# yukiteruono/pbsim3

Measured on AMD Instinct MI355X. Metric: simulated bases/sec, higher is better.
Workload: dtype u8

## Files before the change

pbsim3_amd/csrc/deflate_host.cpp:

```cpp
#include <hip/hip_runtime.h>
#include <limits.h>
#include <math.h>
#include <stdio.h>
#include <stdlib.h>
#include <string.h>

#include <algorithm>
#include <chrono>
#include <functional>
#include <memory>
#include <string>
#include <thread>
#include <vector>

#include "ctx.h"
#include "engine_internal.h"
#include "unit_io.h"

extern "C" {

extern "C++" {
namespace {

int ensure_deflate_tables(pbsim_ctx *c) {
// ... 250 lines not shown
}

}
}

extern "C++" int pbsim::deflate_pieces(pbsim_ctx *c, DfLane &lane, const uint8_t *d_text, int64_t n,
                                       const std::function<int(const char *, int64_t)> &consume,
                                       const std::function<char *(int64_t)> *place, const std::function<bool()> *tail_hook) {
  return deflate_stream(c, lane, d_text, n, consume, place, tail_hook);
}
extern "C++" int pbsim::deflate_handoff(pbsim_ctx *c, DfLane &next, int lane_index, const uint8_t *d_text, int64_t n,
                                        bool own_staging, hipEvent_t text_ready) {
  hipStream_t st = c->df_streams[lane_index][0];
  if (!st || next.own_streams || next.hand_open || n <= 0) return fail("deflate_handoff: bad argument");
  if (!next.ev_hand) HIP_OK(hipEventCreateWithFlags(&next.ev_hand, hipEventDisableTiming));
  HIP_OK(hipStreamWaitEvent(st, text_ready, 0));
  const int ok = df_begin(c, next, d_text, n, own_staging, nullptr);
  if (!ok) next.pre_valid = false;
  next.hand_open = true;
  HIP_OK(hipEventRecord(next.ev_hand, st));
  return ok;
}
extern "C++" int pbsim::deflate_settle(DfLane &lane) {
  if (!lane.hand_open) return PBSIM_SUCCEEDED;
  lane.pre_valid = false;
  HIP_OK(hipEventSynchronize(lane.ev_hand));
  lane.hand_open = false;
  return PBSIM_SUCCEEDED;
}
extern "C++" int pbsim::ensure_deflate_ready(pbsim_ctx *c) {
  for (auto &lane : c->df_streams)
    for (hipStream_t &st : lane)
      if (!st) HIP_OK(hipStreamCreateWithFlags(&st, hipStreamNonBlocking));
  return ensure_deflate_tables(c);
}
extern "C++" int pbsim::ensure_crc_tables(pbsim_ctx *c) { return ensure_deflate_tables(c); }
extern "C++" int pbsim::deflate_prelaunch(pbsim_ctx *c, Slot &sl, bool want_read, bool want_maf) {
  const pbsim_batch_info &bi = sl.b_info;
  if (want_read && bi.read_text_bytes > 0 && !df_begin(c, sl.df[0], sl.d_read_text.as<uint8_t>(), bi.read_text_bytes, true, sl.stream))
    return PBSIM_FAILED;
  if (want_maf && bi.maf_text_bytes > 0 && !df_begin(c, sl.df[1], sl.d_maf_text.as<uint8_t>(), bi.maf_text_bytes, true, sl.stream))
    return PBSIM_FAILED;
  return PBSIM_SUCCEEDED;
}

int pbsim_set_deflate(pbsim_ctx *c, int on) {
  if (!c) return fail("bad argument");
  c->deflate = on & 3;
  c->deflate_parallel = (on & 4) != 0;
  return PBSIM_SUCCEEDED;
}

int64_t pbsim_deflate_bound(int64_t n) {
  if (n <= 0) return 0;
  return n + ((n + DF_CHUNK - 1) / DF_CHUNK) * 31;
}

int pbsim_batch_fetch_deflated(pbsim_ctx *c, char *read_gz, int64_t read_cap, char *maf_gz, int64_t maf_cap,
                               int64_t *read_gz_bytes, int64_t *maf_gz_bytes) {
  if (!c || !c->s().b_finalized) return fail("pbsim_batch_fetch_deflated: no finalized batch");
  NEED_DEVICE(c);
  HIP_OK(hipSetDevice(c->device));
  int64_t nr = 0, nm = 0;
  if (read_gz && !deflate_to_host(c, c->s().df[0], c->s().d_read_text.as<uint8_t>(), c->s().b_info.read_text_bytes, read_gz,
                                  read_cap, &nr))
    return PBSIM_FAILED;
  if (maf_gz && !deflate_to_host(c, c->s().df[0], c->s().d_maf_text.as<uint8_t>(), c->s().b_info.maf_text_bytes, maf_gz,
                                 maf_cap, &nm))
    return PBSIM_FAILED;
  if (read_gz_bytes) *read_gz_bytes = nr;
  if (maf_gz_bytes) *maf_gz_bytes = nm;
  return PBSIM_SUCCEEDED;
}

int pbsim_deflate_buffer(pbsim_ctx *c, const void *src, int64_t n, void *dst, int64_t cap, int64_t *out_bytes) {
  if (!c || !out_bytes || n < 0 || (n > 0 && (!src || !dst))) return fail("pbsim_deflate_buffer: bad argument");
  NEED_DEVICE(c);
  HIP_OK(hipSetDevice(c->device));
  *out_bytes = 0;
  if (n == 0) return PBSIM_SUCCEEDED;
  Slot &sl = c->slots[0];
  DevBuf d_in;
  HIP_OK(d_in.ensure((size_t)n + 16));
  HIP_OK(hipMemcpyAsync(d_in.p, src, (size_t)n, hipMemcpyHostToDevice, sl.stream));
  HIP_OK(hipStreamSynchronize(sl.stream));
  return deflate_to_host(c, sl.df[0], d_in.as<uint8_t>(), n, (char *)dst, cap, out_bytes);
}

extern "C++" int pbsim::deliver(pbsim_ctx *c, const pbsim_sink *sink) {
  const pbsim_batch_info &bi = c->s().b_info;
  if (sink && c->defer_text_sync) {
    NEED_DEVICE(c);
    HIP_OK(hipEventSynchronize(c->s().ev_text));
  }
  if (sink && c->deflate) {
    const bool zr = c->deflate & 1, zm = c->deflate & 2;
    NEED_DEVICE(c);
    HIP_OK(hipSetDevice(c->device));
    if (!zr) HIP_OK(c->s().h_read_text.ensure((size_t)bi.read_text_bytes + 16));
    if (!zm) HIP_OK(c->s().h_maf_text.ensure((size_t)bi.maf_text_bytes + 16));
    if ((!zr || !zm) &&
        !pbsim_batch_fetch(c, zr ? nullptr : (char *)c->s().h_read_text.p, zm ? nullptr : (char *)c->s().h_maf_text.p))
      return PBSIM_FAILED;
    Slot &sl = c->s();
    auto send_read = [&]() -> int {
      if (!(sink->on_read_text && bi.read_text_bytes)) return PBSIM_SUCCEEDED;
      if (!zr)
        return sink->on_read_text(sink->user, (const char *)sl.h_read_text.p, bi.read_text_bytes) ? PBSIM_SUCCEEDED
                                                                                                 : fail("sink aborted (read text)");
      return deflate_stream(c, sl.df[0], sl.d_read_text.as<uint8_t>(), bi.read_text_bytes, [&](const char *z, int64_t k) {
        return sink->on_read_text(sink->user, z, k) ? PBSIM_SUCCEEDED : fail("sink aborted (read text)");
      });
    };
    auto send_maf = [&]() -> int {
      if (!(sink->on_maf_text && bi.maf_text_bytes)) return PBSIM_SUCCEEDED;
      if (!zm)
        return sink->on_maf_text(sink->user, (const char *)sl.h_maf_text.p, bi.maf_text_bytes) ? PBSIM_SUCCEEDED
                                                                                              : fail("sink aborted (MAF text)");
      return deflate_stream(c, sl.df[1], sl.d_maf_text.as<uint8_t>(), bi.maf_text_bytes, [&](const char *z, int64_t k) {
        return sink->on_maf_text(sink->user, z, k) ? PBSIM_SUCCEEDED : fail("sink aborted (MAF text)");
      });
    };
    if (c->deflate_parallel && zr && zm && bi.read_text_bytes && bi.maf_text_bytes) {
      if (!ensure_deflate_tables(c)) return PBSIM_FAILED;
      int ok_read = PBSIM_SUCCEEDED;
      std::string err_read;
      std::thread t([&]() {
        (void)hipSetDevice(c->device);
        ok_read = send_read();
        if (!ok_read) err_read = g_err;
      });
      const int ok_maf = send_maf();
      t.join();
      if (!ok_read) return fail(err_read);
      if (!ok_maf) return PBSIM_FAILED;
    } else {
      if (!send_read()) return PBSIM_FAILED;
      if (!send_maf()) return PBSIM_FAILED;
    }
  } else if (sink) {
    HIP_OK(c->s().h_read_text.ensure((size_t)bi.read_text_bytes + 16));
    HIP_OK(c->s().h_maf_text.ensure((size_t)bi.maf_text_bytes + 16));
    if (!pbsim_batch_fetch(c, (char *)c->s().h_read_text.p, (char *)c->s().h_maf_text.p)) return PBSIM_FAILED;
    if (sink->on_read_text && bi.read_text_bytes &&
        !sink->on_read_text(sink->user, (const char *)c->s().h_read_text.p, bi.read_text_bytes))
      return fail("sink aborted (read text)");
    if (sink->on_maf_text && bi.maf_text_bytes &&
        !sink->on_maf_text(sink->user, (const char *)c->s().h_maf_text.p, bi.maf_text_bytes))
      return fail("sink aborted (MAF text)");
  }
  return c->defer_account ? PBSIM_SUCCEEDED : pbsim_batch_account(c);
}
}
```

pbsim3_amd/csrc/engine_internal.h:

```cpp
#pragma once
#include "ctx.h"

namespace pbsim {
int upload(DevBuf &b, const void *src, size_t n, hipStream_t s);
int ensure_header_tables(pbsim_ctx *c);
int ensure_qs_tabs(pbsim_ctx *c, bool hp11);
int ensure_class_tables(pbsim_ctx *c);
int read_flags(pbsim_ctx *c, DeviceFlags *f);
int prepare_reference(pbsim_ctx *c, uint8_t *d_seq, int64_t len, int keep_first_case, int64_t census_out[kHpSlots]);
int64_t batch_capacity(const pbsim_ctx *c);
int deliver(pbsim_ctx *c, const pbsim_sink *sink);

struct BatchOutput {
  const pbsim_sink *sink;
  const pbsim_array_sink *arrays;
};
int emit_batch(pbsim_ctx *c, const BatchOutput &o, pbsim_batch_info *info);
int deliver_batch(pbsim_ctx *c, const BatchOutput &o);
int simulate_wgs(pbsim_ctx *c, const BatchOutput &out);
int simulate_units_range(pbsim_ctx *c, int64_t first_read, int64_t n_reads, const BatchOutput &out);
int export_batch(pbsim_ctx *c, const pbsim_array_sink *sink, pbsim_batch_info *info);
int deliver_arrays(pbsim_ctx *c, const pbsim_array_sink *sink);

struct DeferTextSync {
  pbsim_ctx *c;
  bool prev;
  explicit DeferTextSync(pbsim_ctx *ctx) : c(ctx), prev(ctx->defer_text_sync) { c->defer_text_sync = true; }
  ~DeferTextSync() {
    for (Slot &sl : c->slots)
      if (sl.stream) (void)hipStreamSynchronize(sl.stream);
    c->defer_text_sync = prev;
  }
};
}
```

pbsim3_amd/csrc/sample.cpp:

```cpp
#include <hip/hip_runtime.h>
#include <limits.h>
#include <math.h>
#include <stdio.h>
#include <stdlib.h>
#include <string.h>

#include <algorithm>
#include <chrono>
#include <functional>
#include <memory>
#include <string>
#include <thread>
#include <vector>

#include "ctx.h"
#include "engine_internal.h"
#include "philox.h"

extern "C" {

int pbsim_set_sample_profile(pbsim_ctx *c, int64_t n, const uint8_t *const *quals, const int64_t *lens) {
  if (!c || n < 1 || !quals || !lens) return fail("pbsim_set_sample_profile: bad argument");
  NEED_DEVICE(c);
  if (c->p.method != PBSIM_METHOD_SAMPLE) return fail("pbsim_set_sample_profile: method is not sample");
// ... 200 lines not shown
    HIP_OK(sl.d_scratch.ensure((size_t)c->scratch_budget + kScratchSlack, true));
    HIP_OK(c->d_sq_line_len.ensure(n_lines * 4));
    HIP_OK(c->d_sq_line_qoff.ensure(n_lines * 8));
    HIP_OK(c->d_sq_vbase.ensure((n_lw + 1) * 4));
    DeviceFlags f0;
    memset(&f0, 0, sizeof f0);
    f0.total_slots = V * 64;
    f0.n_final = n_tasks;
    HIP_OK(hipMemcpyAsync(sl.d_flags.p, &f0, sizeof f0, hipMemcpyHostToDevice, sl.stream));
    HIP_OK(hipMemcpyAsync(c->d_sq_line_len.p, ck.h_len.data(), n_lines * 4, hipMemcpyHostToDevice, sl.stream));
    HIP_OK(hipMemcpyAsync(c->d_sq_line_qoff.p, ck.h_qoff.data(), n_lines * 8, hipMemcpyHostToDevice, sl.stream));
    HIP_OK(hipMemcpyAsync(c->d_sq_vbase.p, ck.h_vbase.data(), (n_lw + 1) * 4, hipMemcpyHostToDevice, sl.stream));
    HIP_OK(hipMemcpyAsync(sl.d_task_of_slot.p, ck.h_tos.data(), V * 64 * 4, hipMemcpyHostToDevice, sl.stream));
    HIP_OK(hipMemcpyAsync(sl.d_slot_of_task.p, ck.h_sot.data(), n_tasks * 4, hipMemcpyHostToDevice, sl.stream));
    HIP_OK(hipMemcpyAsync(sl.d_wave_cap.p, ck.h_cap.data(), V * 4, hipMemcpyHostToDevice, sl.stream));
    HIP_OK(hipMemcpyAsync(sl.d_wave_off.p, ck.h_woff.data(), V * 8, hipMemcpyHostToDevice, sl.stream));
    DeviceFlags *flags = sl.d_flags.as<DeviceFlags>();
    SampleArgs a;
    memset(&a, 0, sizeof a);
    a.seed = c->p.seed;
    a.unit = (uint32_t)c->unit;
    a.first_read = first_read;
    a.n_lines = (int32_t)n_lines;
    a.n_line_waves = (int32_t)n_lw;
    a.n_coop_waves = ck.n_coop_waves;
    {
      constexpr int64_t kCoopBlocksMax = 1024;
      a.n_coop_blocks = (int32_t)std::min<int64_t>(((int64_t)ck.n_coop_waves * 64 + 3) / 4, kCoopBlocksMax);
    }
    a.n_coop_slots = (int64_t)ck.h_vbase[(size_t)ck.n_coop_waves] * 64;
    a.ref.seq = c->d_seq;
    a.ref.hp = c->d_hp.as<uint8_t>();
    a.ref.len = G;
    a.quals = c->d_sq.as<uint8_t>();
    a.line_qoff = c->d_sq_line_qoff.as<int64_t>();
    a.line_len = c->d_sq_line_len.as<int32_t>();
    a.vbase = c->d_sq_vbase.as<int32_t>();
    a.task_of_slot = sl.d_task_of_slot.as<int32_t>();
    a.wave_cap = sl.d_wave_cap.as<int32_t>();
    a.wave_off = sl.d_wave_off.as<int64_t>();
    a.scratch = sl.d_scratch.as<uint8_t>();
    a.span = sl.d_len.as<int32_t>();
    a.off = sl.d_off.as<int32_t>();
    a.out_len = sl.d_out_len.as<int32_t>();
    a.maf_len = sl.d_maf_len.as<int32_t>();
    a.nsub = sl.d_nsub.as<int32_t>();
    a.nins = sl.d_nins.as<int32_t>();
    a.ndel = sl.d_ndel.as<int32_t>();
    a.qsum = sl.d_qsum.as<double>();
    const uint8_t *t = c->d_qs_tabs_v[c->bias.hp11_seen].as<uint8_t>();
    a.sub_thre = reinterpret_cast<const uint32_t *>(t);
    a.ins_thre = reinterpret_cast<const uint32_t *>(t + 94 * 4);
    a.del_thr = reinterpret_cast<const uint32_t *>(t + 94 * 8);
    a.qprob = reinterpret_cast<const double *>(t + 94 * 8 + 94 * 48);
    a.flags = flags;
    if (sl.sq_pending) {
      HIP_OK(hipStreamWaitEvent(sl.stream, sl.ev_sq_done, 0));
      sl.sq_pending = false;
    }
    launch_walk_sample(a, c->seq_hp_flag, sl.stream);
    if (a.n_coop_slots > 0) {
      if (!c->sq_stream) HIP_OK(hipStreamCreateWithFlags(&c->sq_stream, hipStreamNonBlocking));
      if (!sl.ev_sq_walk) {
        HIP_OK(hipEventCreateWithFlags(&sl.ev_sq_walk, hipEventDisableTiming));
        HIP_OK(hipEventCreateWithFlags(&sl.ev_sq_done, hipEventDisableTiming));
      }
      HIP_OK(hipEventRecord(sl.ev_sq_walk, sl.stream));
      HIP_OK(hipStreamWaitEvent(c->sq_stream, sl.ev_sq_walk, 0));
      launch_sample_qsum(a, c->sq_stream);
      HIP_OK(hipEventRecord(sl.ev_sq_done, c->sq_stream));
      sl.sq_pending = true;
    }
    launch_gather_pass0_scan(a.out_len, n_tasks, 1, sl.d_cum.as<int64_t>(), sl.d_scan_tmp.as<int64_t>(),
                             &flags->sums[0], sl.stream);
    HIP_OK(hipGetLastError());
    return PBSIM_SUCCEEDED;
  }
  int finish(const Chunk &ck, int64_t first_read) {
    Slot &sl = c->s();
    const int64_t n_tasks = ck.n_tasks, V = (int64_t)ck.h_cap.size();
    sl.b_enqueued = false;
    DeviceFlags f;
    if (!read_flags(c, &f)) return PBSIM_FAILED;
    if (f.error & kErrScratchOverflow) return fail("a sampled read produced more MAF columns than its scratch holds");
    sl.b_first = first_read;
    sl.b_n = n_tasks;
    sl.b_slots_max = V * 64;
    sl.b_truncated = false;
    sl.b_enqueued = false;
    sl.b_walked = true;
    sl.b_finalized = false;
    sl.b_pass0 = f.sums[0];
    return PBSIM_SUCCEEDED;
  }
  int launch(const Chunk &ck, int64_t first_read) { return enqueue(ck, first_read) && finish(ck, first_read); }
};

int sample_common_checks(pbsim_ctx *c) {
  if (c->p.method != PBSIM_METHOD_SAMPLE) return fail("pbsim_simulate_sample: method is not sample");
  if (!c->d_seq) return fail("no reference set (pbsim_set_reference)");
  if (c->sq_len.empty()) return fail("no sample profile set (pbsim_set_sample_profile)");
  HIP_OK(hipSetDevice(c->device));
  if (!ensure_class_tables(c) || !ensure_qs_tabs(c, c->bias.hp11_seen)) return PBSIM_FAILED;
  return PBSIM_SUCCEEDED;
}

}
}

int pbsim_simulate_sample(pbsim_ctx *c, const pbsim_sink *sink) {
  if (!c) return fail("bad argument");
  NEED_DEVICE(c);
  if (!sample_common_checks(c)) return PBSIM_FAILED;
  pbsim_reset_stats(c);
  const int64_t quota = pbsim_unit_quota(c);
  SampleChunks S;
  S.c = c;
  if (!S.init(quota)) return PBSIM_FAILED;
  const int64_t F = S.F;
  for (int s = 0; s < 2; s++) c->slots[(size_t)s].ref = current_ref(c);
  struct Pos {
    int64_t sv = 0, line = 0;
    bool open = false;
  } pos;
  auto next_chunk = [&](int64_t res_now, Pos *at, SampleChunks::Chunk *ck) -> int {
    for (;;) {
      if (!at->open) {
        at->sv = (int64_t)(header_block(c->p.seed, (uint32_t)c->unit, (uint32_t)(res_now + 1)).w % (uint32_t)F);
        at->line = 0;
        at->open = true;
      }
      while (at->line < F) {
        if (!S.plan(at->sv, at->line, (size_t)1 << 18, ck)) return PBSIM_FAILED;
        if (!ck->cand.empty()) return PBSIM_SUCCEEDED;
        at->line = ck->next_probe;
      }
      S.sample_num = 0;
      S.carry_line = -1;
      at->open = false;
    }
  };
  DeferTextSync defer_guard(c);
  SampleChunks::Chunk cks[2];
  int cur = 0;
  bool have = false;
  const bool trace = getenv("PBSIM_TRACE") != nullptr;
  auto wall_ms = []() {
    struct timespec ts;
    clock_gettime(CLOCK_MONOTONIC, &ts);
    return ts.tv_sec * 1e3 + ts.tv_nsec * 1e-6;
  };
  int64_t len_total = 0, res = 0;
  bool done = false;
  auto drain = [&]() {
    for (int s = 0; s < 2; s++)
      if (c->slots[(size_t)s].stream) (void)hipStreamSynchronize(c->slots[(size_t)s].stream);
    c->cur = 0;
  };
  while (len_total < quota && !done) {
    SampleChunks::Chunk &ck = cks[cur];
    c->cur = cur;
    if (!have) {
      const double t0 = trace ? wall_ms() : 0;
      if (!next_chunk(res, &pos, &ck)) {
        drain();
        return PBSIM_FAILED;
      }
      const double t1 = trace ? wall_ms() : 0;
      if (!S.enqueue(ck, res + 1)) {
        drain();
        return PBSIM_FAILED;
      }
      if (trace) fprintf(stderr, "[pbsim sample] chunk of %zu strings, %lld reads: planned in %.2f ms, enqueued in %.2f ms\n", ck.n_c, (long long)ck.n_tasks, t1 - t0, wall_ms() - t1);
    }
    have = false;
    const SampleChunks::Ent last = ck.cand[ck.n_c - 1];
    int64_t last_done = 0;
    const bool last_unfinished = S.last_unfinished(pos.sv, ck, &last_done);
    if (!S.finish(ck, res + 1)) {
      drain();
      return PBSIM_FAILED;
    }
    pbsim_batch_info bi;
    if (!pbsim_batch_finalize(c, len_total, &bi)) {
      drain();
      return PBSIM_FAILED;
    }
    bool look = !last_unfinished && bi.n_final == ck.n_tasks && bi.len_total_after < quota;
    if (look && c->slots[(size_t)(1 - cur)].d_scratch.bytes < (size_t)c->scratch_budget) {
      size_t free_b = 0, total_b = 0;
      HIP_OK(hipMemGetInfo(&free_b, &total_b));
      const double text_now = (double)c->s().d_read_text.bytes + (double)c->s().d_maf_text.bytes;
      if ((double)free_b < 1.1 * (double)c->scratch_budget + 1.5 * text_now + (double)(2ull << 30)) look = false;
    }
    Pos pos2 = pos;
    if (look) {
      S.carry_line = -1;
      S.carry_done = 0;
      pos2.line = last.line + 1;
      c->cur = 1 - cur;
      if (!next_chunk(res + bi.n_final, &pos2, &cks[1 - cur]) || !S.enqueue(cks[1 - cur], res + bi.n_final + 1)) {
        drain();
        return PBSIM_FAILED;
      }
      c->cur = cur;
    }
    if (!deliver(c, sink)) {
      drain();
      return PBSIM_FAILED;
    }
    len_total = bi.len_total_after;
    res += bi.n_final;
    if (bi.n_final < ck.n_tasks) done = true;
    if (look) {
      pos = pos2;
      cur = 1 - cur;
      have = true;
      continue;
    }
    if (last_unfinished && !done) {
      S.carry_line = last.line;
      S.carry_done = last_done;
      HIP_OK(hipMemcpy(&S.carry_len, c->s().d_out_len.as<int32_t>() + (ck.n_tasks - 1), 4, hipMemcpyDeviceToHost));
      pos.line = last.line;
    } else {
      S.carry_line = -1;
      S.carry_done = 0;
      pos.line = last.line + 1;
    }
  }
  if (have) {
    drain();
    return fail("internal: a sampled chunk was left in flight");
  }
  c->cur = 0;
  return PBSIM_SUCCEEDED;
}

static int sample_comm_run(pbsim_ctx *c, const pbsim_comm *comm, const pbsim_record_sink *sink, bool *agreed) {
  const int W = comm->world, rank = comm->rank;
  int ok = sample_common_checks(c);
  SampleChunks S;
  S.c = c;
  const int64_t quota = ok ? pbsim_unit_quota(c) : 0;
  if (ok) ok = S.init(quota);
  {
    std::string keep = g_err;
    int64_t v[2] = {ok ? 0 : 1, -c->scratch_budget};
    if (!comm->all_reduce_i64(comm->user, v, 2, PBSIM_OP_MAX)) return fail("pbsim_comm.all_reduce_i64 failed");
    if (v[0]) {
      *agreed = true;
      return ok ? fail("another rank failed") : fail(keep);
    }
    c->scratch_budget = -v[1];
  }
  pbsim_reset_stats(c);
  c->st.keep_values = true;
  c->cur = 0;
  Slot &sl = c->s();
  sl.ref = current_ref(c);
  const int64_t F = S.F;
  int64_t len_total = 0, res = 0, read_off = 0, maf_off = 0;
  bool done = false;
  std::vector<SampleChunks::Chunk> cks((size_t)W);
  std::string buf_r, buf_m;
  struct Keep {
    std::string *r, *m;
  } keep = {&buf_r, &buf_m};
  const pbsim_sink collect = {&keep,
                              [](void *u, const char *t, int64_t k) { ((Keep *)u)->r->append(t, (size_t)k); return 1; },
                              [](void *u, const char *t, int64_t k) { ((Keep *)u)->m->append(t, (size_t)k); return 1; }};
  auto gather = [&](const int64_t *send, int n, std::vector<int64_t> *recv) -> int {
    recv->assign((size_t)W * n, 0);
    return comm->all_gather_i64(comm->user, send, n, recv->data()) ? PBSIM_SUCCEEDED : fail("pbsim_comm.all_gather_i64 failed");
  };
  std::vector<int64_t> A, B, Cs;
  const bool trace = getenv("PBSIM_TRACE") != nullptr;
  while (len_total < quota && !done) {
    const int64_t sv = (int64_t)(header_block(c->p.seed, (uint32_t)c->unit, (uint32_t)(res + 1)).w % (uint32_t)F);
    int64_t line = 0;
    while (line < F && len_total < quota && !done) {
      const int64_t left = S.count_candidates(sv, line);
      if (left == 0) break;
      const size_t per = (size_t)std::min<int64_t>((left + W - 1) / W, (int64_t)1 << 18);
      int n_chunks = 0;
      int64_t at = line, first = res + 1, my_first = 0;
      int local = PBSIM_SUCCEEDED;
      std::string local_err;
      for (int q = 0; q < W && at < F; q++) {
        SampleChunks::Chunk &ck = cks[(size_t)q];
        if (!S.plan(sv, at, per, &ck)) {
          local = PBSIM_FAILED;
          local_err = g_err;
          break;
        }
        if (ck.cand.empty()) break;
        int64_t last_done = 0;
        if (S.last_unfinished(sv, ck, &last_done)) {
          local = PBSIM_FAILED;
          local_err = "the copies of one sampled read do not fit a rank's scratch pool: the sharded sampling method needs a larger "
                      "pool (pbsim_set_scratch_bytes / PBSIM_SCRATCH_MB), or run this profile on one GPU";
          break;
        }
        if (q == rank) my_first = first;
        first += ck.n_tasks;
        at = ck.cand[ck.n_c - 1].line + 1;
        n_chunks++;
      }
      if (!local) {
        *agreed = true;
        return fail(local_err);
      }
      const bool mine = rank < n_chunks;
      if (trace)
        fprintf(stderr, "[pbsim sample r%d] sweep sv=%lld line=%lld left=%lld chunks=%d first=%lld len_total=%lld\n", rank, (long long)sv,
                (long long)line, (long long)left, n_chunks, (long long)(res + 1), (long long)len_total);
      int64_t sendA[2] = {0, 0};
      if (mine) {
        if (S.launch(cks[(size_t)rank], my_first)) sendA[0] = sl.b_pass0;
        else sendA[1] = 1, local_err = g_err;
      }
      if (!gather(sendA, 2, &A)) return PBSIM_FAILED;
      int64_t before = len_total, bad = 0;
      for (int q = 0; q < W; q++) {
        bad += A[(size_t)q * 2 + 1];
        if (q < rank) before += A[(size_t)q * 2];
      }
      if (bad) {
        *agreed = true;
        return sendA[1] ? fail(local_err) : fail("another rank failed");
      }
      pbsim_batch_info bi;
      memset(&bi, 0, sizeof bi);
      int64_t sendB[3] = {0, before, 0};
      if (mine) {
        if (finalize_cut(c, before, &bi)) sendB[0] = bi.n_final, sendB[1] = bi.len_total_after;
        else sendB[2] = 1, local_err = g_err;
      }
      if (!gather(sendB, 3, &B)) return PBSIM_FAILED;
      bad = 0;
      for (int q = 0; q < W; q++) bad += B[(size_t)q * 3 + 2];
      if (bad) {
        *agreed = true;
        return sendB[2] ? fail(local_err) : fail("another rank failed");
      }
      int cut = -1;
      for (int q = 0; q < n_chunks && cut < 0; q++)
        if (B[(size_t)q * 3] < cks[(size_t)q].n_tasks) cut = q;
      const int last_valid = cut < 0 ? n_chunks - 1 : cut;
      buf_r.clear();
      buf_m.clear();
      int64_t sendC[3] = {0, 0, 0};
      if (mine && rank <= last_valid && bi.n_final > 0) {
        if (finalize_text(c, &bi) && deliver(c, &collect)) sendC[0] = (int64_t)buf_r.size(), sendC[1] = (int64_t)buf_m.size();
        else sendC[2] = 1, local_err = g_err;
      }
      if (!gather(sendC, 3, &Cs)) return PBSIM_FAILED;
      bad = 0;
      int64_t r_at = read_off, m_at = maf_off;
      for (int q = 0; q < W; q++) {
        bad += Cs[(size_t)q * 3 + 2];
        if (q < rank) r_at += Cs[(size_t)q * 3], m_at += Cs[(size_t)q * 3 + 1];
        read_off += Cs[(size_t)q * 3];
        maf_off += Cs[(size_t)q * 3 + 1];
      }
      if (bad) {
        *agreed = true;
        return sendC[2] ? fail(local_err) : fail("another rank failed");
      }
      if (sink && sink->on_read_text && !buf_r.empty() && !sink->on_read_text(sink->user, c->unit, buf_r.data(), (int64_t)buf_r.size(), r_at))
        return fail("sink aborted (read text)");
      if (sink && sink->on_maf_text && !buf_m.empty() && !sink->on_maf_text(sink->user, c->unit, buf_m.data(), (int64_t)buf_m.size(), m_at))
        return fail("sink aborted (MAF text)");
      for (int q = 0; q <= last_valid; q++) res += B[(size_t)q * 3];
      len_total = B[(size_t)last_valid * 3 + 1];
      if (cut >= 0) done = true;
      line = cks[(size_t)last_valid].cand[cks[(size_t)last_valid].n_c - 1].line + 1;
      if (trace)
        fprintf(stderr, "[pbsim sample r%d]   round done: cut=%d res=%lld len_total=%lld next line=%lld\n", rank, cut, (long long)res,
                (long long)len_total, (long long)line);
    }
    S.sample_num = 0;
  }
  int64_t extra[2] = {0, 0};
  if (!stats_merge(&c->st, c->p, comm, extra, 0)) return PBSIM_FAILED;
  c->st.keep_values = false;
  if (sink && sink->on_record_done) {
// ... 24 lines not shown
```

pbsim3_amd/csrc/units.cpp:

```cpp
#include <ctype.h>
#include <hip/hip_runtime.h>
#include <limits.h>
#include <math.h>
#include <stdio.h>
#include <stdlib.h>
#include <string.h>

#include <algorithm>
#include <chrono>
#include <functional>
#include <future>
#include <memory>
#include <string>
#include <thread>
#include <vector>

#include "ctx.h"
#include "engine_internal.h"
#include "input_file.h"
#include "unit_io.h"
#include "philox.h"

extern "C" {

// ... 48 lines not shown
        const int64_t off = offt[(size_t)u * 21 + ssp[(size_t)urank[u] * 1000 + w.z % (rv ? rv : 1u)]];
        if (off + L > lens[u]) L = lens[u] - off;
        runit.push_back((int32_t)u);
        rbase.push_back(pos);
        rminus.push_back((i > plus_exp[u]) ? 1 : 0);
        if (acc == 100) i = std::max<int64_t>(L, 0);
        continue;
      }
      runit.push_back((int32_t)u);
      rbase.push_back(pos);
      rminus.push_back((i > plus_exp[u]) ? 1 : 0);
    }
    pos += lens[u] + 1;
  }
  reads = (int64_t)runit.size();

  hp_bias_default(&c->bias);
  c->bias.hp11_seen = false;
  if (c->p.hp_del_bias != 1) {
    int64_t freq[kHpSlots] = {0};
    for (int64_t u = 0; u < n; u++)
      hp_census_weighted(seqs[u], lens[u], (int64_t)(int)(plus_exp[u] + minus_exp[u]), keep_first, freq);
    hp_bias_from_census(c->p.hp_del_bias, freq, &c->bias);
    c->bias.hp11_seen = freq[11] > 0;
  }
  c->class_tables_dirty = true;
  c->coop_wg_errhmm[0] = c->coop_wg_errhmm[1] = 0;

  HIP_OK(c->d_seq_own.ensure((size_t)total + 64));
  HIP_OK(hipMemcpyAsync(c->d_seq_own.p, cat.data(), (size_t)total, hipMemcpyHostToDevice, c->stream));
  HIP_OK(hipMemsetAsync(c->d_seq_own.as<uint8_t>() + total, 0, 64, c->stream));
  int64_t census[kHpSlots] = {0};
  if (!prepare_reference(c, c->d_seq_own.as<uint8_t>(), total, keep_first, census)) return PBSIM_FAILED;
  memcpy(c->unit_census, census, sizeof census);
  if (reads > 0) {
    if (!upload(c->d_read_unit, runit.data(), runit.size() * 4, c->stream)) return PBSIM_FAILED;
    if (!upload(c->d_read_base, rbase.data(), rbase.size() * 8, c->stream)) return PBSIM_FAILED;
    if (!upload(c->d_read_minus, rminus.data(), rminus.size(), c->stream)) return PBSIM_FAILED;
  }
  if (!upload(c->d_unit_len, ulen.data(), ulen.size() * 8, c->stream)) return PBSIM_FAILED;
  if (!upload(c->d_unit_rank, urank.data(), urank.size() * 4, c->stream)) return PBSIM_FAILED;
  if (!upload(c->d_unit_names, names.data(), names.size(), c->stream)) return PBSIM_FAILED;
  if (!upload(c->d_off_table, offt.data(), offt.size() * 4, c->stream)) return PBSIM_FAILED;
  if (!upload(c->d_ssp, ssp.data(), ssp.size(), c->stream)) return PBSIM_FAILED;
  if (!upload(c->d_ssp_rv, st.rv.data(), st.rv.size() * 4, c->stream)) return PBSIM_FAILED;
  HIP_OK(hipStreamSynchronize(c->stream));
  c->d_seq = c->d_seq_own.as<uint8_t>();
  c->ref_len = total;
  c->unit = 0;
  c->n_units = n;
  c->trans_reads = reads;
  c->unit_sn.clear();
  c->unit_ln.assign(lens, lens + n);
  for (int64_t u = 0; u < n; u++) {
    const char *nm = &names[(size_t)u * 132];
    size_t k = 0;
    while (nm[k] && !isspace((unsigned char)nm[k])) k++;
    c->unit_sn.emplace_back(nm, k);
  }
  for (Slot &sl : c->slots) sl.b_enqueued = sl.b_walked = sl.b_finalized = false;
  return PBSIM_SUCCEEDED;
}

int pbsim_set_transcripts(pbsim_ctx *c, int64_t n, const char *const *ids, const int64_t *plus_exp,
                          const int64_t *minus_exp, const uint8_t *const *seqs, const int64_t *lens) {
  if (!c || n < 1 || !ids || !plus_exp || !minus_exp || !seqs || !lens) return fail("pbsim_set_transcripts: bad argument");
  NEED_DEVICE(c);
  if (c->p.strategy != PBSIM_STRATEGY_TRANS) return fail("pbsim_set_transcripts: strategy is not trans");
  return set_units(c, n, ids, plus_exp, minus_exp, seqs, lens, false);
}

int pbsim_set_templates(pbsim_ctx *c, int64_t n, const char *const *ids, const uint8_t *const *seqs,
                        const int64_t *lens) {
  if (!c || n < 1 || !ids || !seqs || !lens) return fail("pbsim_set_templates: bad argument");
  NEED_DEVICE(c);
  if (c->p.strategy != PBSIM_STRATEGY_TEMPL) return fail("pbsim_set_templates: strategy is not templ");
  std::vector<int64_t> one((size_t)n, 1), zero((size_t)n, 0);
  return set_units(c, n, ids, one.data(), zero.data(), seqs, lens, true);
}

int pbsim_simulate_templ(pbsim_ctx *c, const pbsim_sink *sink) { return pbsim_simulate_trans(c, sink); }

int pbsim_simulate_trans(pbsim_ctx *c, const pbsim_sink *sink) {
  if (!c) return fail("bad argument");
  return pbsim_simulate_units_range(c, 1, c->trans_reads, sink);
}

int64_t pbsim_unit_reads(pbsim_ctx *c) { return c ? c->trans_reads : -1; }

static int load_unit_file(pbsim_ctx *c, const char *path, int64_t stats[2], bool templ) {
  if (!c || !path) return fail("bad argument");
  std::vector<Transcript> tr;
  std::string err;
  long a = 0;
  long long b = 0;
  pbsim_ctx *const was = set_input_context(c);
  const bool ok = templ ? read_templates(path, &tr, &a, &b, &err) : read_transcripts(path, &tr, &a, &err);
  set_input_context(was);
  if (!ok) return fail(err);
  std::vector<const char *> ids;
  std::vector<int64_t> plus, minus, lens;
  std::vector<const uint8_t *> seqs;
  for (auto &t : tr) {
    ids.push_back(t.id.c_str());
    plus.push_back(t.plus);
    minus.push_back(t.minus);
    seqs.push_back((const uint8_t *)t.seq.data());
    lens.push_back((int64_t)strlen(t.seq.c_str()));
  }
  if (stats) {
    stats[0] = templ ? (int64_t)a : (int64_t)tr.size();
    stats[1] = templ ? (int64_t)b : (int64_t)a;
  }
  return templ ? pbsim_set_templates(c, (int64_t)tr.size(), ids.data(), seqs.data(), lens.data())
               : pbsim_set_transcripts(c, (int64_t)tr.size(), ids.data(), plus.data(), minus.data(), seqs.data(), lens.data());
}
int pbsim_load_transcript_file(pbsim_ctx *c, const char *path, int64_t stats[2]) { return load_unit_file(c, path, stats, false); }
int pbsim_load_template_file(pbsim_ctx *c, const char *path, int64_t stats[2]) { return load_unit_file(c, path, stats, true); }

int pbsim_simulate_units_range(pbsim_ctx *c, int64_t first_read, int64_t n_reads, const pbsim_sink *sink) {
  if (!c) return fail("bad argument");
  return simulate_units_range(c, first_read, n_reads, BatchOutput{sink, nullptr});
}

extern "C++" int pbsim::simulate_units_range(pbsim_ctx *c, int64_t first_read, int64_t n_reads, const BatchOutput &out) {
  const pbsim_sink *sink = out.sink;
  NEED_DEVICE(c);
  if (c->p.strategy == PBSIM_STRATEGY_WGS) return fail("pbsim_simulate_trans: strategy is wgs");
  if (!c->d_seq || c->n_units < 1) return fail("no transcripts/templates set");
  if (first_read < 1 || n_reads < 0 || first_read - 1 + n_reads > c->trans_reads)
    return fail("pbsim_simulate_units_range: reads outside 1 .. pbsim_unit_reads()");
  pbsim_reset_stats(c);
  DeferTextSync defer_guard(c);
  const bool delivering = sink && c->deflate != 0 && (sink->on_read_text || sink->on_maf_text);
  const int n_slots = delivering ? std::max(3, kPipelineDepth) : kPipelineDepth;
  const int64_t R = first_read - 1 + n_reads;
  int64_t cap = batch_capacity(c);
  struct Pending {
    int slot;
    int64_t first, n;
  };
  std::vector<Pending> fifo;
  auto drop_pending = [&]() {
    for (const Pending &pd : fifo) {
      c->cur = pd.slot;
      (void)hipStreamSynchronize(c->s().stream);
      c->s().b_enqueued = false;
    }
    fifo.clear();
    c->cur = 0;
  };
  const int n_parts = n_slots;
  const bool prelaunch = delivering && (c->deflate & 3) == 3;
  int64_t next_begin = first_read, next_read = first_read;
  int next_slot = 0;
  bool have_prev = false;
  int prev_slot = 0;
  struct DeferAccount {
    pbsim_ctx *c;
    bool was;
    DeferAccount(pbsim_ctx *cc, bool on) : c(cc), was(cc->defer_account) { c->defer_account = on; }
    ~DeferAccount() { c->defer_account = was; }
  } account_guard(c, delivering);
  std::future<int> acct;
  auto join_acct = [&]() -> int {
    if (!acct.valid()) return PBSIM_SUCCEEDED;
    return acct.get() ? PBSIM_SUCCEEDED : fail("the statistics of a batch could not be added");
  };
  auto deliver_prev = [&]() -> int {
    if (!have_prev) return PBSIM_SUCCEEDED;
    have_prev = false;
    c->cur = prev_slot;
    return deliver_batch(c, out);
  };
  auto give_up = [&]() {
    if (acct.valid()) (void)acct.get();
    drop_pending();
    if (have_prev) {
      c->cur = prev_slot;
      (void)hipStreamSynchronize(c->s().stream);
      have_prev = false;
      c->cur = 0;
    }
  };
  while (next_read <= R) {
    while ((int)fifo.size() + (have_prev ? 1 : 0) < n_slots && next_begin <= R) {
      const int64_t part = std::max<int64_t>(65536, (n_reads + n_parts - 1) / n_parts);
      const int64_t n = std::min(std::min(cap, part), R - next_begin + 1);
      c->cur = next_slot;
      if (!pbsim_batch_walk_begin(c, next_begin, n, -1)) {
        give_up();
        return PBSIM_FAILED;
      }
      fifo.push_back(Pending{next_slot, next_begin, n});
      next_slot = (next_slot + 1) % n_slots;
      next_begin += n;
    }
    if (fifo.empty()) {
      if (!deliver_prev()) {
        give_up();
        return PBSIM_FAILED;
      }
      continue;
    }
    const Pending pd = fifo.front();
    fifo.erase(fifo.begin());
    c->cur = pd.slot;
    if (!pbsim_batch_walk_end(c, nullptr)) {
      const bool budget = g_err.rfind("scratch budget exceeded", 0) == 0 && pd.n > 1;
      const std::string keep = g_err;
      drop_pending();
      if (!budget) {
        give_up();
        g_err = keep;
        return PBSIM_FAILED;
      }
      cap = std::max<int64_t>(1, pd.n / 2);
      next_begin = pd.first;
      next_slot = have_prev ? (prev_slot + 1) % n_slots : 0;
      continue;
    }
    pbsim_batch_info bi;
    if (!finalize_cut(c, 0, &bi) || !emit_batch(c, out, &bi)) {
      give_up();
      return PBSIM_FAILED;
    }
    next_read += bi.n_final;
    if (prelaunch && !deflate_prelaunch(c, c->s(), sink->on_read_text != nullptr, sink->on_maf_text != nullptr)) {
      give_up();
      return PBSIM_FAILED;
    }
    if (delivering) {
      if (!join_acct()) {
        give_up();
        return PBSIM_FAILED;
      }
      Slot *sl = &c->s();
      acct = std::async(std::launch::async, [c, sl]() { return account_of(c, *sl, &c->st); });
    }
    if (!deliver_prev()) {
      give_up();
      return PBSIM_FAILED;
    }
    have_prev = true;
    prev_slot = pd.slot;
  }
  if (!deliver_prev() || !join_acct()) {
    give_up();
    return PBSIM_FAILED;
  }
  return PBSIM_SUCCEEDED;
}

}
```

Baseline: 57.70 billion.

## Deliver compressed read and MAF text on two background lane threads

Adds a UnitDelivery class with two worker threads, one for read text and one for MAF text. Each thread compresses and hands its batch's text to the sink while the main loop goes on simulating later batches. Slots are reused only after both lanes have finished with them, and a lane can start the deflate head of the next batch while finishing the tail of the current one. This aims to take per-batch delivery and compression off the critical path of the simulation loop, at the cost of extra threads, locking and more complex failure handling.

```diff
diff --git a/pbsim3_amd/csrc/deflate_host.cpp b/pbsim3_amd/csrc/deflate_host.cpp
--- a/pbsim3_amd/csrc/deflate_host.cpp
+++ b/pbsim3_amd/csrc/deflate_host.cpp
@@ -426,3 +426,99 @@
   return c->defer_account ? PBSIM_SUCCEEDED : pbsim_batch_account(c);
 }
 }
+
+namespace pbsim {
+
+bool UnitDelivery::wanted(const pbsim_ctx *c, const pbsim_sink *sink) {
+  const char *e = getenv("PBSIM_UNIT_LANES");
+  return sink && sink->on_read_text && sink->on_maf_text && c->deflate == 3 && c->deflate_parallel && !(e && atoi(e) == 0);
+}
+
+int UnitDelivery::start() {
+  if (!ensure_deflate_ready(c_)) return PBSIM_FAILED;
+  started_ = true;
+  th_[0] = std::thread([this]() { lane_main(0); });
+  th_[1] = std::thread([this]() { lane_main(1); });
+  return PBSIM_SUCCEEDED;
+}
+
+void UnitDelivery::lane_main(int which) {
+  (void)hipSetDevice(c_->device);
+  int64_t handed_seq = -1;
+  UnitBatch b;
+  while (q_.next(which, &b)) {
+    const std::function<bool()> hook = [&]() -> bool {
+      UnitBatch nx;
+      if (!q_.peek(which, &nx)) return false;
+      if (nx.seq <= handed_seq) return true;
+      handed_seq = nx.seq;
+      if (!nx.text[which] || nx.bytes[which] <= 0) return true;
+      if (deflate_handoff(c_, c_->slots[(size_t)nx.slot].df[which], which, (const uint8_t *)nx.text[which], nx.bytes[which], true,
+                          (hipEvent_t)nx.ev_text))
+        handed_[which]++;
+      return true;
+    };
+    int ok = PBSIM_SUCCEEDED;
+    if (b.text[which] && b.bytes[which] > 0) {
+      if (hipEventSynchronize((hipEvent_t)b.ev_text) != hipSuccess) ok = fail("the text emission of a batch failed");
+      if (ok)
+        ok = deflate_stream(c_, c_->slots[(size_t)b.slot].df[which], (const uint8_t *)b.text[which], b.bytes[which],
+                            [&](const char *z, int64_t k) {
+                              if (q_.failed()) return fail("delivery stopped: the other stream failed");
+                              if (which == 0)
+                                return sink_->on_read_text(sink_->user, z, k) ? PBSIM_SUCCEEDED : fail("sink aborted (read text)");
+                              return sink_->on_maf_text(sink_->user, z, k) ? PBSIM_SUCCEEDED : fail("sink aborted (MAF text)");
+                            },
+                            nullptr, &hook);
+    }
+    if (!ok) {
+      q_.fail(g_err);
+      return;
+    }
+    q_.done(which);
+  }
+}
+
+int64_t UnitDelivery::post(int slot) {
+  const Slot &sl = c_->slots[(size_t)slot];
+  UnitBatch b;
+  b.slot = slot;
+  b.text[0] = sl.d_read_text.p;
+  b.text[1] = sl.d_maf_text.p;
+  b.bytes[0] = sl.b_info.read_text_bytes;
+  b.bytes[1] = sl.b_info.maf_text_bytes;
+  b.ev_text = sl.ev_text;
+  const int64_t seq = q_.post(b);
+  if (seq < 0) (void)fail(q_.failed() ? q_.error() : std::string("internal: a batch posted to closed delivery lanes"));
+  return seq;
+}
+
+int UnitDelivery::wait_done(int64_t seq) { return q_.wait_done(seq) ? PBSIM_SUCCEEDED : fail(q_.error()); }
+
+void UnitDelivery::join() {
+  if (!started_ || joined_) return;
+  for (std::thread &t : th_)
+    if (t.joinable()) t.join();
+  joined_ = true;
+}
+
+int UnitDelivery::finish() {
+  q_.close();
+  join();
+  return q_.failed() ? fail(q_.error()) : PBSIM_SUCCEEDED;
+}
+
+void UnitDelivery::abort() {
+  if (!started_ || (joined_ && !q_.failed())) return;
+  const std::string keep = g_err;
+  q_.fail(keep);
+  join();
+  for (auto &lane : c_->df_streams)
+    for (hipStream_t st : lane)
+      if (st) (void)hipStreamSynchronize(st);
+  for (Slot &sl : c_->slots)
+    for (DfLane &L : sl.df) (void)deflate_settle(L);
+  g_err = keep;
+}
+
+}
diff --git a/pbsim3_amd/csrc/engine_internal.h b/pbsim3_amd/csrc/engine_internal.h
--- a/pbsim3_amd/csrc/engine_internal.h
+++ b/pbsim3_amd/csrc/engine_internal.h
@@ -1,5 +1,8 @@
 #pragma once
+#include <thread>
+
 #include "ctx.h"
+#include "unit_lanes.h"
 
 namespace pbsim {
 int upload(DevBuf &b, const void *src, size_t n, hipStream_t s);
@@ -22,6 +25,30 @@
 int export_batch(pbsim_ctx *c, const pbsim_array_sink *sink, pbsim_batch_info *info);
 int deliver_arrays(pbsim_ctx *c, const pbsim_array_sink *sink);
 
+class UnitDelivery {
+ public:
+  static bool wanted(const pbsim_ctx *c, const pbsim_sink *sink);
+  UnitDelivery(pbsim_ctx *c, const pbsim_sink *sink) : c_(c), sink_(sink) {}
+  ~UnitDelivery() { abort(); }
+  int start();
+  int64_t post(int slot);
+  int wait_done(int64_t seq);
+  int64_t done_count() { return q_.done_count(); }
+  int finish();
+  void abort();
+  int64_t heads_handed() const { return handed_[0] + handed_[1]; }
+
+ private:
+  void lane_main(int which);
+  void join();
+  pbsim_ctx *c_;
+  const pbsim_sink *sink_;
+  UnitLanes q_;
+  std::thread th_[2];
+  int64_t handed_[2] = {0, 0};
+  bool started_ = false, joined_ = false;
+};
+
 struct DeferTextSync {
   pbsim_ctx *c;
   bool prev;
diff --git a/pbsim3_amd/csrc/sample.cpp b/pbsim3_amd/csrc/sample.cpp
--- a/pbsim3_amd/csrc/sample.cpp
+++ b/pbsim3_amd/csrc/sample.cpp
@@ -376,7 +376,18 @@
   };
   int64_t len_total = 0, res = 0;
   bool done = false;
+  const bool lanes = UnitDelivery::wanted(c, sink);
+  std::unique_ptr<UnitDelivery> ud;
+  int64_t seq_of[2] = {-1, -1};
+  const bool trace_job = trace || getenv("PBSIM_DEFLATE_TRACE");
+  if (trace_job) fprintf(stderr, "[pbsim unit job] entered at %.3f ms (%s)\n", wall_ms(), lanes ? "delivery lanes" : "caller delivers");
+  if (lanes) {
+    ud.reset(new UnitDelivery(c, sink));
+    if (!ud->start()) return PBSIM_FAILED;
+  }
+  auto slot_free = [&](int s) -> int { return !ud || seq_of[s] < 0 || ud->wait_done(seq_of[s]); };
   auto drain = [&]() {
+    if (ud) ud->abort();
     for (int s = 0; s < 2; s++)
       if (c->slots[(size_t)s].stream) (void)hipStreamSynchronize(c->slots[(size_t)s].stream);
     c->cur = 0;
@@ -391,7 +402,7 @@
         return PBSIM_FAILED;
       }
       const double t1 = trace ? wall_ms() : 0;
-      if (!S.enqueue(ck, res + 1)) {
+      if (!slot_free(cur) || !S.enqueue(ck, res + 1)) {
         drain();
         return PBSIM_FAILED;
       }
@@ -417,19 +428,24 @@
       const double text_now = (double)c->s().d_read_text.bytes + (double)c->s().d_maf_text.bytes;
       if ((double)free_b < 1.1 * (double)c->scratch_budget + 1.5 * text_now + (double)(2ull << 30)) look = false;
     }
+    if (lanes && (seq_of[cur] = ud->post(cur)) < 0) {
+      drain();
+      return PBSIM_FAILED;
+    }
     Pos pos2 = pos;
     if (look) {
       S.carry_line = -1;
       S.carry_done = 0;
       pos2.line = last.line + 1;
       c->cur = 1 - cur;
-      if (!next_chunk(res + bi.n_final, &pos2, &cks[1 - cur]) || !S.enqueue(cks[1 - cur], res + bi.n_final + 1)) {
+      if (!slot_free(1 - cur) || !next_chunk(res + bi.n_final, &pos2, &cks[1 - cur]) ||
+          !S.enqueue(cks[1 - cur], res + bi.n_final + 1)) {
         drain();
         return PBSIM_FAILED;
       }
       c->cur = cur;
     }
-    if (!deliver(c, sink)) {
+    if (lanes ? !account_of(c, c->slots[(size_t)cur], &c->st) : !deliver(c, sink)) {
       drain();
       return PBSIM_FAILED;
     }
@@ -457,6 +473,12 @@
     drain();
     return fail("internal: a sampled chunk was left in flight");
   }
+  if (ud && !ud->finish()) {
+    drain();
+    return PBSIM_FAILED;
+  }
+  if (trace_job)
+    fprintf(stderr, "[pbsim unit job] returns at %.3f ms; %lld lane heads launched at a tail\n", wall_ms(), (long long)(ud ? ud->heads_handed() : 0));
   c->cur = 0;
   return PBSIM_SUCCEEDED;
 }
diff --git a/pbsim3_amd/csrc/unit_lanes.h b/pbsim3_amd/csrc/unit_lanes.h
--- /dev/null
+++ b/pbsim3_amd/csrc/unit_lanes.h
@@ -0,0 +1,96 @@
+#pragma once
+#include <stdint.h>
+
+#include <condition_variable>
+#include <deque>
+#include <mutex>
+#include <string>
+
+namespace pbsim {
+
+struct UnitBatch {
+  int64_t seq = -1;
+  int slot = -1;
+  const void *text[2] = {nullptr, nullptr};
+  int64_t bytes[2] = {0, 0};
+  void *ev_text = nullptr;
+};
+
+class UnitLanes {
+ public:
+  int64_t post(UnitBatch b) {
+    {
+      std::lock_guard<std::mutex> lk(mu_);
+      if (failed_ || closed_) return -1;
+      b.seq = posted_++;
+      q_[0].push_back(b);
+      q_[1].push_back(b);
+    }
+    cv_.notify_all();
+    return b.seq;
+  }
+  bool wait_done(int64_t seq) {
+    std::unique_lock<std::mutex> lk(mu_);
+    cv_.wait(lk, [&] { return failed_ || (done_[0] > seq && done_[1] > seq); });
+    return !failed_;
+  }
+  int64_t done_count() {
+    std::lock_guard<std::mutex> lk(mu_);
+    return done_[0] < done_[1] ? done_[0] : done_[1];
+  }
+  void close() {
+    {
+      std::lock_guard<std::mutex> lk(mu_);
+      closed_ = true;
+    }
+    cv_.notify_all();
+  }
+  void fail(const std::string &why) {
+    {
+      std::lock_guard<std::mutex> lk(mu_);
+      if (!failed_) err_ = why;
+      failed_ = true;
+    }
+    cv_.notify_all();
+  }
+  bool failed() {
+    std::lock_guard<std::mutex> lk(mu_);
+    return failed_;
+  }
+  std::string error() {
+    std::lock_guard<std::mutex> lk(mu_);
+    return err_;
+  }
+
+  bool next(int lane, UnitBatch *b) {
+    std::unique_lock<std::mutex> lk(mu_);
+    cv_.wait(lk, [&] { return failed_ || closed_ || !q_[lane].empty(); });
+    if (failed_ || q_[lane].empty()) return false;
+    *b = q_[lane].front();
+    q_[lane].pop_front();
+    return true;
+  }
+  bool peek(int lane, UnitBatch *b) {
+    std::lock_guard<std::mutex> lk(mu_);
+    if (failed_ || q_[lane].empty()) return false;
+    *b = q_[lane].front();
+    return true;
+  }
+  void done(int lane) {
+    {
+      std::lock_guard<std::mutex> lk(mu_);
+      done_[lane]++;
+    }
+    cv_.notify_all();
+  }
+
+ private:
+  std::mutex mu_;
+  std::condition_variable cv_;
+  std::deque<UnitBatch> q_[2];
+  int64_t posted_ = 0, done_[2] = {0, 0};
+  bool closed_ = false, failed_ = false;
+  std::string err_;
+};
+
+}
diff --git a/pbsim3_amd/csrc/units.cpp b/pbsim3_amd/csrc/units.cpp
--- a/pbsim3_amd/csrc/units.cpp
+++ b/pbsim3_amd/csrc/units.cpp
@@ -224,6 +224,19 @@
   };
   const int n_parts = n_slots;
   const bool prelaunch = delivering && (c->deflate & 3) == 3;
+  const bool lanes = delivering && !out.arrays && UnitDelivery::wanted(c, sink);
+  std::unique_ptr<UnitDelivery> ud;
+  int64_t slot_seq[kMaxSlots];
+  std::fill(slot_seq, slot_seq + kMaxSlots, (int64_t)-1);
+  int64_t n_posted = 0;
+  bool lanes_idle = true;
+  const bool trace_job = getenv("PBSIM_TRACE") || getenv("PBSIM_DEFLATE_TRACE");
+  const auto now_ms = []() { return std::chrono::duration<double, std::milli>(std::chrono::steady_clock::now().time_since_epoch()).count(); };
+  if (trace_job) fprintf(stderr, "[pbsim unit job] entered at %.3f ms (%s)\n", now_ms(), lanes ? "delivery lanes" : "caller delivers");
+  if (lanes) {
+    ud.reset(new UnitDelivery(c, sink));
+    if (!ud->start()) return PBSIM_FAILED;
+  }
   int64_t next_begin = first_read, next_read = first_read;
   int next_slot = 0;
   bool have_prev = false;
@@ -246,6 +259,7 @@
     return deliver_batch(c, out);
   };
   auto give_up = [&]() {
+    if (ud) ud->abort();
     if (acct.valid()) (void)acct.get();
     drop_pending();
     if (have_prev) {
@@ -257,6 +271,7 @@
   };
   while (next_read <= R) {
     while ((int)fifo.size() + (have_prev ? 1 : 0) < n_slots && next_begin <= R) {
+      if (lanes && slot_seq[next_slot] >= ud->done_count()) break;
       const int64_t part = std::max<int64_t>(65536, (n_reads + n_parts - 1) / n_parts);
       const int64_t n = std::min(std::min(cap, part), R - next_begin + 1);
       c->cur = next_slot;
@@ -267,6 +282,13 @@
       fifo.push_back(Pending{next_slot, next_begin, n});
       next_slot = (next_slot + 1) % n_slots;
       next_begin += n;
+    }
+    if (fifo.empty() && lanes) {
+      if (!ud->wait_done(slot_seq[next_slot])) {
+        give_up();
+        return PBSIM_FAILED;
+      }
+      continue;
     }
     if (fifo.empty()) {
       if (!deliver_prev()) {
@@ -290,6 +312,14 @@
       cap = std::max<int64_t>(1, pd.n / 2);
       next_begin = pd.first;
       next_slot = have_prev ? (prev_slot + 1) % n_slots : 0;
+      if (lanes) {
+        if (n_posted > 0 && !ud->wait_done(n_posted - 1)) {
+          give_up();
+          return PBSIM_FAILED;
+        }
+        std::fill(slot_seq, slot_seq + kMaxSlots, (int64_t)-1);
+        lanes_idle = true;
+      }
       continue;
     }
     pbsim_batch_info bi;
@@ -298,7 +328,7 @@
       return PBSIM_FAILED;
     }
     next_read += bi.n_final;
-    if (prelaunch && !deflate_prelaunch(c, c->s(), sink->on_read_text != nullptr, sink->on_maf_text != nullptr)) {
+    if (prelaunch && (!lanes || lanes_idle) && !deflate_prelaunch(c, c->s(), sink->on_read_text != nullptr, sink->on_maf_text != nullptr)) {
       give_up();
       return PBSIM_FAILED;
     }
@@ -310,17 +340,33 @@
       Slot *sl = &c->s();
       acct = std::async(std::launch::async, [c, sl]() { return account_of(c, *sl, &c->st); });
     }
-    if (!deliver_prev()) {
+    if (lanes) {
+      if ((slot_seq[pd.slot] = ud->post(pd.slot)) < 0) {
+        give_up();
+        return PBSIM_FAILED;
+      }
+      n_posted++;
+      lanes_idle = false;
+      continue;
+    }
+    if (delivering && !deliver_prev()) {
       give_up();
       return PBSIM_FAILED;
     }
     have_prev = true;
     prev_slot = pd.slot;
-  }
-  if (!deliver_prev() || !join_acct()) {
+    if (!delivering && !deliver_prev()) {
+      give_up();
+      return PBSIM_FAILED;
+    }
+  }
+  if (!deliver_prev() || (ud && !ud->finish()) || !join_acct()) {
     give_up();
     return PBSIM_FAILED;
   }
+  if (trace_job)
+    fprintf(stderr, "[pbsim unit job] returns at %.3f ms; %lld batches, %lld lane heads launched at a tail\n", now_ms(), (long long)n_posted,
+            (long long)(ud ? ud->heads_handed() : 0));
   return PBSIM_SUCCEEDED;
 }
 
```

Measured after the change: 55.52 billion. 3.8% lower.
